# hellovuong/ORB_SLAM3_FAST

Hardware: AMD Instinct MI355X
Metric: ORB extract+match frames/sec @1280×720 stereo (both-eye ORBextractor + ComputeStereoMatches) (higher is better)
Workload: dtype u8; 1 GPU; C3: synthetic 1280x720 rectified stereo pairs, 1500 features, 8 levels, scale 1.2, FAST 20/7, ComputeStereoMatches (bf=0.12*532.03, b=0.12); handles=4, distinct_streams_per_gpu=32, frames_in_ring=3, stereo_matches_pair0=987, parallelism=independent stereo pairs sharded across GPUs, no data-path collective

## Files before the change

### include/orbx.h

```cpp
#ifndef ORBX_H_
#define ORBX_H_

#include <stddef.h>
#include <stdint.h>

#ifdef __cplusplus
extern "C" {
#endif

#define ORBX_MAX_LEVELS 12

#define ORBX_OK 0
#define ORBX_E_EMPTY (-1)
#define ORBX_E_BADARG (-2)
#define ORBX_E_CAPACITY (-3)
#define ORBX_E_HIP (-4)
#define ORBX_E_NODEVICE (-5)
#define ORBX_E_UNSUPPORTED (-6)
#define ORBX_E_TIMEOUT (-7)

typedef struct orbx_keypoint {
  float x, y, size, angle, response;
  int32_t octave, class_id;
} orbx_keypoint;
// ... 576 lines not shown
int orbx_copy_probe(int device, size_t bytes, int iters, double* gbps);

void orbx_debug_introsort(uint64_t* v, int n);
int orbx_debug_introsort_device(int device, uint64_t* v, int n);

void orbx_debug_set_detect_list_cap(int cap);
void orbx_debug_set_octree_global(int on);
void orbx_debug_set_stereo_direct(int max_pairs);
int orbx_debug_upload_results(orbx_extractor* ex, int image, const orbx_keypoint* kps, const uint8_t* desc, int n, int mono_index);
void orbx_debug_set_clahe_cell_kernel(int on);
void orbx_debug_set_remap_lds(int on);
int orbx_debug_remap_footprints(const float* map_x, const float* map_y, ptrdiff_t map_stride, int out_w, int out_h, int src_w,
                                int src_h, int n_maps, int32_t* table, int cap, int32_t* tiles_x, int32_t* tiles_y);
int orbx_debug_front_tables(const orbx_params* p, int width, int height, uint32_t* cells, int cells_cap, uint32_t* tiles,
                            int tiles_cap, int32_t info[4]);
int orbx_debug_preproc_plan(const orbx_preproc* pp, int32_t info[8]);
void orbx_debug_set_resize_tail(int first_level, int max_levels, int band_rows);
int orbx_debug_resize_plan(const orbx_extractor* ex, int32_t* first_level, int32_t* n_levels, int32_t* n_bands, int cap);
int orbx_debug_score_map(orbx_extractor* ex, int enable);
int orbx_debug_score_level(orbx_extractor* ex, int image, int level, uint8_t* dst, ptrdiff_t dst_stride);
int orbx_debug_sincos(int device, const float* angles, int n, int fused, float* sin_out, float* cos_out);

#ifdef __cplusplus
}
#endif
#endif
```

### orb_slam3_fast_amd/__init__.py

```python
import ctypes as C
import os

import numpy as np

_HERE = os.path.dirname(os.path.abspath(__file__))
LIB_PATH = os.path.join(_HERE, os.environ.get("ORBX_LIB_NAME", "liborbx.so"))

KP_DTYPE = np.dtype([("x", "<f4"), ("y", "<f4"), ("size", "<f4"), ("angle", "<f4"), ("response", "<f4"),
                     ("octave", "<i4"), ("class_id", "<i4")])
assert KP_DTYPE.itemsize == 28

OK, E_EMPTY, E_BADARG, E_CAPACITY, E_HIP, E_NODEVICE, E_UNSUPPORTED, E_TIMEOUT = 0, -1, -2, -3, -4, -5, -6, -7
TH_HIGH, TH_LOW, HISTO_LENGTH = 100, 50, 30
NUM_STAGES = 8
MP_DTYPE = np.dtype([("proj_x", "<f4"), ("proj_y", "<f4"), ("proj_xr", "<f4"), ("view_cos", "<f4"), ("track_depth", "<f4"),
                     ("predicted_level", "<i4"), ("in_view", "u1"), ("bad", "u1"), ("has_observations", "u1"),
                     ("pad_", "u1"), ("desc", "u1", (32,))])
assert MP_DTYPE.itemsize == 60
PP_DTYPE = np.dtype([("u", "<f4"), ("v", "<f4"), ("ur", "<f4"), ("radius", "<f4"), ("angle", "<f4"), ("min_level", "<i4"),
                     ("max_level", "<i4"), ("valid", "u1"), ("has_observations", "u1"), ("pad_", "u1", (2,)),
                     ("desc", "u1", (32,))])
assert PP_DTYPE.itemsize == 64
FP_DTYPE = np.dtype([("u", "<f4"), ("v", "<f4"), ("ur", "<f4"), ("radius", "<f4"), ("predicted_level", "<i4"), ("valid", "u1"),
                     ("pad_", "u1", (3,)), ("desc", "u1", (32,))])
# ... 170 lines not shown
        L.orbx_debug_set_detect_list_cap.argtypes = [i]
        L.orbx_debug_set_detect_list_cap.restype = None
        L.orbx_debug_set_octree_global.argtypes = [i]
        L.orbx_debug_set_octree_global.restype = None
        L.orbx_debug_set_stereo_direct.argtypes = [i]
        L.orbx_debug_set_stereo_direct.restype = None
        L.orbx_debug_set_clahe_cell_kernel.argtypes = [i]
        L.orbx_debug_set_clahe_cell_kernel.restype = None
        L.orbx_debug_upload_results.argtypes = [vp, i, vp, vp, i, i]
        L.orbx_debug_set_remap_lds.argtypes = [i]
        L.orbx_debug_set_remap_lds.restype = None
        L.orbx_debug_remap_footprints.argtypes = [vp, vp, C.c_ssize_t, i, i, i, i, i, vp, i, C.POINTER(i), C.POINTER(i)]
        L.orbx_debug_preproc_plan.argtypes = [vp, vp]
        if hasattr(L, "orbx_debug_front_tables"):
            L.orbx_debug_front_tables.argtypes = [vp, i, i, vp, i, vp, i, vp]
        L.orbx_debug_set_resize_tail.argtypes = [i, i, i]
        L.orbx_debug_set_resize_tail.restype = None
        L.orbx_debug_resize_plan.argtypes = [vp, vp, vp, vp, i]
        L.orbx_debug_sincos.argtypes = [i, vp, i, i, vp, vp]
        L.orbx_debug_score_map.argtypes = [vp, i]
        L.orbx_set_opencv_compat.argtypes = [vp, i]
        L.orbx_debug_score_level.argtypes = [vp, i, i, vp, C.c_ssize_t]
        _lib = L
    return _lib


def _check(rc):
    if rc < 0:
        raise OrbxError(rc, lib().orbx_last_error().decode())
    return rc
# ... 1090 lines not shown
        raise OrbxError("unexpected tile grid %d x %d" % (gx.value, gy.value))
    return tab if rc == 1 else None


def front_tables(nfeatures, scaleFactor, nlevels, iniThFAST, minThFAST, width, height):
    prm = _Params(int(nfeatures), float(scaleFactor), int(nlevels), int(iniThFAST), int(minThFAST))
    info = np.zeros(4, np.int32)
    _check(lib().orbx_debug_front_tables(C.byref(prm), width, height, None, 0, None, 0, _p(info)))
    cells = np.zeros((int(info[0]), 16), np.uint32)
    tiles = np.zeros(int(info[1]), np.uint32)
    _check(lib().orbx_debug_front_tables(C.byref(prm), width, height, _p(cells), cells.size, _p(tiles) if tiles.size else None,
                                         tiles.size, _p(info)))
    return cells, tiles, int(info[2]), int(info[3])


class ORBVocabulary:

    def __init__(self, k=None, L=None, parent=None, is_leaf=None, desc=None, weight=None, scoring=0, weighting=0, path=None,
                 device=0):
        h = C.c_void_p()
        if path is not None:
            _check(lib().orbx_vocabulary_load_text(device, path.encode(), C.byref(h)))
        else:
            parent = np.ascontiguousarray(parent, np.int32)
            leaf = np.ascontiguousarray(is_leaf, np.uint8)
            d = np.ascontiguousarray(desc, np.uint8)
            w = np.ascontiguousarray(weight, np.float64)
            _check(lib().orbx_vocabulary_create(device, k, L, scoring, weighting, len(parent), _p(parent), _p(leaf), _p(d), _p(w),
                                                C.byref(h)))
        self._h = h
# ... 491 lines not shown
```

### orb_slam3_fast_amd/csrc/orbx_api.hip

```cpp
#include "orbx_host.h"
#include "orbx_rgbd.h"

namespace orbx_host {
thread_local std::string g_err;
}

namespace {
struct StageTimer {
  orbx_extractor* ex;
  hipStream_t s;
  int stage;
  size_t i0 = 0;
  bool on;
  StageTimer(orbx_extractor* ex_, hipStream_t s_, int stage_)
      : ex(ex_), s(s_), stage(stage_), on(ex_->profiling && (ex_->profStage < 0 || ex_->profStage == stage_)) {
    if (!on) {
      if (s == ex->stream) ex->lastEvValid = false;
      return;
    }
    if (s == ex->stream && ex->lastEvValid) {
      i0 = ex->lastEv;
    } else {
      hipEvent_t e = ex->next_event();
      i0 = ex->evCursor - 1;
// ... 175 lines not shown
        t[3] = (uint32_t)cb | ((uint32_t)ndw << 16);
        t[4] = (fast ? kTileFast : 0u) | (whole ? kTileWhole : 0u);
        t[5] = (uint32_t)((long long)y0 * D.pitch);
        t[6] = (uint32_t)tby;
      }
      for (int w = 0; w < 4; w++)
        for (int k = 0; k < 4; k++) {
          const int dy = std::min(y0 + w + 4 * k, D.h - 1);
          const uint32_t sy = yrow[D.ycoef + dy];
          uint32_t* r = &tab[(size_t)rowOff + 16 * (size_t)(4 * tby + w) + 4 * k];
          r[0] = (uint32_t)(uint16_t)yab[2 * (D.ycoef + dy)] | ((uint32_t)(uint16_t)yab[2 * (D.ycoef + dy) + 1] << 16);
          r[1] = (uint32_t)(((int)(sy & 0xFFFFu) - rb) * 512);
          r[2] = (uint32_t)(((int)(sy >> 16) - rb) * 512);
        }
    }
  }
}

void build_cell_records(const Geom& g, std::vector<CellRec>& recs) {
  recs.assign((size_t)g.totalCells, CellRec{});
  const int TPd = g.tileP >> 2;
  for (int l = 0; l < g.nlevels; l++) {
    const LevelDev& L = g.lv[l];
    const int maxBX = L.w - kBorder, maxBY = L.h - kBorder;
    for (int ci = 0; ci < L.nRows; ci++)
      for (int cj = 0; cj < L.nCols; cj++) {
        const int cell = ci * L.nCols + cj;
        CellRec& r = recs[(size_t)L.cellStart + cell];
        const int iniY = kBorder + ci * L.hCell, iniX = kBorder + cj * L.wCell;
        const int maxY = std::min(iniY + L.hCell + 6, maxBY), maxX = std::min(iniX + L.wCell + 6, maxBX);
// ... 225 lines not shown
  g.cellImg = m.cellImg;
  std::vector<uint4> xtab;
  std::vector<int> yofs;
  std::vector<short> yab;
  build_coefs(g, xtab, yofs, yab);
  HIPC(hipStreamSynchronize(ex->stream));
  HIPC(hipMemcpy(ex->d_xtab.p, xtab.data(), xtab.size() * sizeof(uint4), hipMemcpyHostToDevice));
  HIPC(hipMemcpy(ex->d_yofs.p, yofs.data(), yofs.size() * sizeof(int), hipMemcpyHostToDevice));
  {
    std::vector<uint32_t> yrow, rec;
    build_yrow(g, yofs, yrow);
    HIPC(hipMemcpy(ex->d_yrow.p, yrow.data(), yrow.size() * sizeof(uint32_t), hipMemcpyHostToDevice));
    build_resize_records(g, xtab, yrow, yab, rec);
    if (ex->d_rsRec.n < rec.size()) HIPC(ex->d_rsRec.alloc(rec.size()));
    if (!rec.empty()) HIPC(hipMemcpy(ex->d_rsRec.p, rec.data(), rec.size() * sizeof(uint32_t), hipMemcpyHostToDevice));
  }
  HIPC(hipMemcpy(ex->d_yab.p, yab.data(), yab.size() * sizeof(short), hipMemcpyHostToDevice));
  {
    std::vector<CellRec> recs;
    build_cell_records(g, recs);
    HIPC(hipMemcpy(ex->d_cellRec.p, recs.data(), recs.size() * sizeof(CellRec), hipMemcpyHostToDevice));
  }
  HIPC(prepare_kernels(g));
  std::vector<TailPlan> plans;
  std::vector<TailBand> bands;
  build_tail_plans(g, yofs, plans, bands);
  if (!plans.empty()) {
    if (ex->d_tailBands.n < bands.size()) HIPC(ex->d_tailBands.alloc(bands.size()));
    HIPC(hipMemcpy(ex->d_tailBands.p, bands.data(), bands.size() * sizeof(TailBand), hipMemcpyHostToDevice));
    unsigned lds = 0;
// ... 92 lines not shown
  if (ex->useLat) {
    for (const TailPlan& tp : ex->latTails) {
      StageTimer t(ex, s, ORBX_STAGE_RESIZE);
      HIPC(launch_resize_tail(g, ex->pyr, tp, ex->d_latBands.p + tp.bandOff, img0, n, ex->d_xtab.p, ex->d_yofs.p, ex->d_yab.p, s));
    }
    return ORBX_OK;
  }
  size_t seg = 0;
  for (int l = 1; l < g.nlevels;) {
    StageTimer t(ex, s, ORBX_STAGE_RESIZE);
    if (seg < ex->tails.size() && ex->tails[seg].lA == l) {
      const TailPlan& tp = ex->tails[seg++];
      HIPC(launch_resize_tail(g, ex->pyr, tp, ex->d_tailBands.p + tp.bandOff, 0, n, ex->d_xtab.p, ex->d_yofs.p, ex->d_yab.p, s));
      l += tp.nT;
    } else {
      HIPC(launch_resize(g, ex->pyr, n, l, ex->d_xtab.p, ex->d_yrow.p, ex->d_yab.p, ex->d_rsRec.p, s));
      l++;
    }
  }
  return ORBX_OK;
}

int enqueue_extract(orbx_extractor* ex, const uint8_t* d_images, int n, int w, int h, ptrdiff_t row_pitch,
                    ptrdiff_t image_pitch, const int32_t* lap) {
  bool lapTrivial = true;
  int rc = prepare_extract(ex, d_images, n, w, h, row_pitch, image_pitch, lap, lapTrivial);
  if (rc != ORBX_OK) return rc;
  hipStream_t s = ex->stream;
  static const bool useGraph = getenv("ORBX_GRAPH") && atoi(getenv("ORBX_GRAPH")) != 0;
  if (useGraph && n == 1 && d_images == ex->d_stage.p && !ex->profiling && !ex->graphOff) {
    if (ex->graphW != w || ex->graphH != h) {
// ... 822 lines not shown
  build_yrow(g, yofs, yrow);
  build_resize_records(g, xtab, yrow, yab, rec);
  build_cell_records(g, cr);
  info[0] = (int32_t)cr.size(); info[1] = (int32_t)rec.size(); info[2] = g.tileP; info[3] = g.tileH;
  if (cells) {
    if (cr.size() * 16 > (size_t)cells_cap) return fail(ORBX_E_CAPACITY, "cell records larger than cells_cap");
    std::memcpy(cells, cr.data(), cr.size() * sizeof(CellRec));
  }
  if (tiles) {
    if (rec.size() > (size_t)tiles_cap) return fail(ORBX_E_CAPACITY, "tile records larger than tiles_cap");
    std::memcpy(tiles, rec.data(), rec.size() * sizeof(uint32_t));
  }
  return ORBX_OK;
}

int orbx_hamming256(const void* a, const void* b) {
  const uint32_t* x = (const uint32_t*)a;
  const uint32_t* y = (const uint32_t*)b;
  int d = 0;
  for (int i = 0; i < 8; i++) d += __builtin_popcount(x[i] ^ y[i]);
  return d;
}

static int enqueue_stereo_match(orbx_extractor* left, int first_left, orbx_extractor* right, int first_right,
                                int n_pairs, float bf, float b, bool withFilter, StereoArgs* argsOut,
                                const ResultPack* packWithBand, bool* packedOut) {
  if (packedOut) *packedOut = false;
  if (!left || !right) return fail(ORBX_E_BADARG, "null handle");
  if (n_pairs <= 0 || first_left < 0 || first_right < 0 || first_left + n_pairs > left->lastN ||
      first_right + n_pairs > right->lastN)
// ... 355 lines not shown
```

### orb_slam3_fast_amd/csrc/orbx_host.h

```cpp
#ifndef ORBX_HOST_H
#define ORBX_HOST_H
#if defined(__x86_64__) || defined(__i386__)
#include <immintrin.h>
static inline void cpu_pause() { _mm_pause(); }
#else
static inline void cpu_pause() {}
#endif
#include <memory>
#include <new>
#include <chrono>
#include <cmath>
#include <cstdio>
#include <cstdlib>
#include <cstring>
#include <string>
#include <mutex>
#include <vector>

#include "orbx_internal.h"

using namespace orbx;

namespace orbx_host {


extern thread_local std::string g_err;
void build_coefs(const Geom& g, std::vector<uint4>& xtab, std::vector<int>& yofs, std::vector<short>& yab);
void build_cell_records(const Geom& g, std::vector<CellRec>& recs);
void build_yrow(const Geom& g, const std::vector<int>& yofs, std::vector<uint32_t>& yrow);
void build_resize_records(const Geom& g, const std::vector<uint4>& xtab, const std::vector<uint32_t>& yrow, const std::vector<short>& yab,
                          std::vector<uint32_t>& tab);
inline int fail(int code, const std::string& msg) {
  g_err = msg;
  return code;
}
inline double trace_slow_ms() {
  static const double v = getenv("ORBX_TRACE_SLOW") ? atof(getenv("ORBX_TRACE_SLOW")) : 0.0;
  return v;
}
#define HIPC(expr)                                                                                     \
  do {                                                                                                 \
    const double lim_ = trace_slow_ms();                                                               \
    const auto t0_ = lim_ > 0 ? std::chrono::steady_clock::now() : std::chrono::steady_clock::time_point(); \
    hipError_t e_ = (expr);                                                                            \
    if (lim_ > 0) {                                                                                    \
      const double ms_ = std::chrono::duration<double, std::milli>(std::chrono::steady_clock::now() - t0_).count(); \
// ... 236 lines not shown
  std::vector<int> nfeat;
  int umax[16];
  Geom g{};
  Geom gmax{};
  int curW = 0, curH = 0;
  Pyr pyr{};
  int lastN = 0;
  DevBuf<uint8_t> d_pyr, d_blur, d_stage, d_desc;
  DevBuf<uint8_t> d_dbgScore;
  DevBuf<uint32_t> d_cand, d_cellCand, d_sel;
  DevBuf<uint16_t> d_knode;
  DevBuf<int> d_rowStart, d_cellCount, d_cellPrefix, d_candCount, d_selCount, d_slot, d_nOut, d_mono, d_lap, d_yofs, d_sad;
  DevBuf<short> d_yab;
  DevBuf<uint4> d_xtab;
  DevBuf<uint32_t> d_rsRec;
  DevBuf<orbx::CellRec> d_cellRec;
  DevBuf<int> d_packCtr;
  uint32_t packSeq = 0;
  bool packCtrDirty = false;
  DevBuf<uint32_t> d_yrow;
  DevBuf<uint4> d_srec, d_sdesc;
  std::vector<orbx::TailPlan> tails;
  DevBuf<orbx::TailBand> d_tailBands;
  std::vector<orbx::TailPlan> latTails;
  DevBuf<orbx::TailBand> d_latBands;
  DevBuf<orbx_keypoint> d_kps;
  DevBuf<float> d_uR, d_depth;
  int stagePitch = 0;
  int stereoPairs = 0;
  int lastStereoPairs = 0;
// ... 94 lines not shown
```

### orb_slam3_fast_amd/csrc/orbx_internal.h

```cpp
#pragma once
#include <hip/hip_runtime.h>
#include <stdint.h>
#include <vector>

#include "../../include/orbx.h"

namespace orbx {

constexpr int kEdge = 19;
constexpr int kHalfPatch = 15;
constexpr int kBorder = 16;
constexpr int kMaxIni = 8;

struct LevelDev {
  int w, h, pitch;
  int nCols, nRows, wCell, hCell;
  int cellStart;
  int quota;
  int candCap;
  int cellCap;
  int selOff, selCap;
  int xcoef, ycoef;
  long long off;
  long long candOff;
// ... 76 lines not shown
  int pitch[ORBX_MAX_LEVELS + 1];
  int rtOff[ORBX_MAX_LEVELS];
  int rtTotal;
  unsigned ldsBytes;
};
hipError_t launch_resize_tail(const Geom& g, const Pyr& p, const TailPlan& tp, const TailBand* bands, int img0, int nimg,
                              const uint4* xtab, const int* yofs, const short* yab, hipStream_t s);
hipError_t prepare_resize_tail(unsigned ldsBytes);
hipError_t raise_dynamic_lds(const void* fn, size_t bytes);

size_t resize_plain_lds(int sw, int sh, int dw, int dh);
hipError_t prepare_resize_plain(int sw, int sh, int dw, int dh);
hipError_t launch_resize_plain(const uint8_t* src, int sw, int sh, long long sp, long long sip, uint8_t* dst, int dw, int dh,
                               long long dp, long long dip, const uint4* xtab, const uint32_t* yrow, const short* yab, int nimg,
                               hipStream_t s);
hipError_t launch_resize(const Geom& g, const Pyr& p, int nimg, int level, const uint4* xtab, const uint32_t* yofs ,
                         const short* yab, const uint32_t* records, hipStream_t s);
int resize_records_layout(const Geom& g, int level, int& tileOff, int& rowOff);
constexpr uint32_t kTileFast = 1u, kTileWhole = 2u;
hipError_t launch_detect(const Geom& g, const Pyr& p, const CellRec* cellRec, int nimg, uint32_t* cellCand, int* cellCount,
                         int level0, int level1, uint8_t* dbgScore, hipStream_t s);
hipError_t launch_octree(const Geom& g, int nimg, const uint32_t* cellCand, const int* cellCount, int* cellPrefix,
                         uint32_t* cand, int* candCount, uint16_t* knode, uint32_t* sel, int* selCount, int level0,
                         int level1, hipStream_t s);
hipError_t launch_blur(const Geom& g, const Pyr& p, int nimg, int level0, int level1, hipStream_t s);
hipError_t launch_slots(const Geom& g, int nimg, const uint32_t* sel, const int* selCount, const int* lap,
                        int* slot, int* nOut, int* mono, hipStream_t s);
hipError_t launch_describe(const Geom& g, const Pyr& p, int nimg, const uint32_t* sel, const int* selCount,
                           const int* slot, orbx_keypoint* kps, uint8_t* desc, int* nOut, int* mono, hipStream_t s);
size_t octree_lds_bytes(const Geom& g);
size_t resize_lds_bytes(const Geom& g);

struct StereoArgs {
// ... 381 lines not shown
```

### orb_slam3_fast_amd/csrc/orbx_kernels.hip

```cpp
#include <type_traits>
#include <map>
#include <mutex>

#include "orbx_device.h"
#include "orbx_introsort.h"
#include "orbx_sincos.h"
#include "orbx_blur_mfma.h"

namespace orbx {

__constant__ int c_umax[16] = {15, 15, 15, 15, 14, 14, 14, 13, 13, 12, 11, 10, 9, 8, 6, 3};

#define RS_DW 256
#define RS_DR 16
#define RS_HROWS 6
struct ResizeLv {
  struct { int w, h, pitch, xcoef, ycoef; } D;
  struct { int w, h; } S;
  int sp, l;
  int nbx;
  const uint8_t* src; long long srcImg;
  uint8_t* dst; long long dstImg;
  const uint32_t* tiles;
  const uint32_t* rows;
};
constexpr int kResizeXcdRun = 8;
__device__ __forceinline__ uint32_t vblend4(uint2 t0, uint2 t1, uint32_t bb, uint32_t kRound) {
  uint32_t p0, p1, p2, p3, q0, q1, q2, q3, w01, w23;
  asm("v_mad_u32_u16 %0, %1, %2, %3" : "=v"(p0) : "v"(t0.x), "s"(bb), "v"(kRound));
  asm("v_mad_u32_u16 %0, %1, %2, %3 op_sel:[1,0,0,0]" : "=v"(p1) : "v"(t0.x), "s"(bb), "v"(kRound));
  asm("v_mad_u32_u16 %0, %1, %2, %3" : "=v"(p2) : "v"(t0.y), "s"(bb), "v"(kRound));
  asm("v_mad_u32_u16 %0, %1, %2, %3 op_sel:[1,0,0,0]" : "=v"(p3) : "v"(t0.y), "s"(bb), "v"(kRound));
  asm("v_mad_u32_u16 %0, %1, %2, 0 op_sel:[0,1,0,0]" : "=v"(q0) : "v"(t1.x), "s"(bb));
  asm("v_mad_u32_u16 %0, %1, %2, 0 op_sel:[1,1,0,0]" : "=v"(q1) : "v"(t1.x), "s"(bb));
  asm("v_mad_u32_u16 %0, %1, %2, 0 op_sel:[0,1,0,0]" : "=v"(q2) : "v"(t1.y), "s"(bb));
  asm("v_mad_u32_u16 %0, %1, %2, 0 op_sel:[1,1,0,0]" : "=v"(q3) : "v"(t1.y), "s"(bb));
  asm("v_add_u32_sdwa %0, %1, %2 dst_sel:WORD_0 dst_unused:UNUSED_PAD src0_sel:WORD_1 src1_sel:WORD_1" : "=v"(w01) : "v"(p0), "v"(q0));
  asm("v_add_u32_sdwa %0, %1, %2 dst_sel:WORD_1 dst_unused:UNUSED_PRESERVE src0_sel:WORD_1 src1_sel:WORD_1" : "+v"(w01) : "v"(p1), "v"(q1));
  asm("v_add_u32_sdwa %0, %1, %2 dst_sel:WORD_0 dst_unused:UNUSED_PAD src0_sel:WORD_1 src1_sel:WORD_1" : "=v"(w23) : "v"(p2), "v"(q2));
  asm("v_add_u32_sdwa %0, %1, %2 dst_sel:WORD_1 dst_unused:UNUSED_PRESERVE src0_sel:WORD_1 src1_sel:WORD_1" : "+v"(w23) : "v"(p3), "v"(q3));
  asm("v_pk_lshrrev_b16 %0, 2, %1 op_sel_hi:[0,1]" : "=v"(w01) : "v"(w01));
  asm("v_pk_lshrrev_b16 %0, 2, %1 op_sel_hi:[0,1]" : "=v"(w23) : "v"(w23));
  return __builtin_amdgcn_perm(w23, w01, 0x06040200u);
}
template <int NDW, bool TAB>
__global__ __launch_bounds__(256) void k_resize(ResizeLv rl, const uint4* __restrict__ xtab,
                                                const uint32_t* __restrict__ yrow, const short* __restrict__ yab,
                                                int srcRowsMax, int srcDwMaxRt) {
  extern __shared__ __attribute__((aligned(16))) uint8_t smem[];
  const int SDW = NDW ? NDW : srcDwMaxRt;
  const auto D = rl.D;
  const auto S = rl.S;
  const int l = rl.l;
  const int tid = threadIdx.x;
  const int img = blockIdx.z;
  const int tIdx = xcd_run_remap<kResizeXcdRun>((int)blockIdx.x, (int)gridDim.x, (int)blockIdx.z);
  const int sp = rl.sp;
  const uint8_t* src = rl.src + (long long)img * rl.srcImg;
  uint32_t* st = reinterpret_cast<uint32_t*>(smem);
  uint8_t* ht8 = smem + (size_t)srcRowsMax * SDW * 4;
#ifdef RS_PROF
  long long tq0 = wall_clock64();
#endif
  const int qc = tid & 63, w = __builtin_amdgcn_readfirstlane(tid >> 6);
  int x0, rowsHere;
  int rb, nrows, cb, ndw;
  bool whole, fastGeom;
  const uint4* xt;
  uint8_t* dstTile;
  uint32_t vbb[RS_DR / 4];
  int vr0[RS_DR / 4], vr1[RS_DR / 4];
  constexpr int kFastTrips = 8;
  if (TAB) {
    const uint32_t* tr = rl.tiles + 8 * tIdx;
    xt = xtab + tr[0];
    x0 = (int)(tr[1] & 0xFFFFu), rowsHere = (int)(tr[1] >> 16);
    rb = (int)(tr[2] & 0xFFFFu), nrows = (int)(tr[2] >> 16);
    cb = (int)(tr[3] & 0xFFFFu), ndw = (int)(tr[3] >> 16);
    whole = (tr[4] & kTileWhole) != 0, fastGeom = (tr[4] & kTileFast) != 0;
    dstTile = rl.dst + (long long)img * rl.dstImg + tr[5];
    const uint4* rw4 = reinterpret_cast<const uint4*>(rl.rows) + (4 * (int)tr[6] + w) * (RS_DR / 4);
#pragma unroll
    for (int k = 0; k < RS_DR / 4; k++) {
      const uint4 e = rw4[k];
      vbb[k] = e.x, vr0[k] = (int)e.y, vr1[k] = (int)e.z;
    }
  } else {
    const int tby = __builtin_amdgcn_readfirstlane((int)(((float)tIdx + 0.5f) * __builtin_amdgcn_rcpf((float)rl.nbx)));
    const int tbx = tIdx - tby * rl.nbx;
    const int y0 = tby * RS_DR;
    x0 = tbx * RS_DW;
    const int x1 = min(x0 + RS_DW, D.w) - 1, y1 = min(y0 + RS_DR, D.h) - 1;
    rowsHere = y1 - y0 + 1;
    rb = (int)(yrow[D.ycoef + y0] & 0xFFFFu);
    nrows = (int)(yrow[D.ycoef + y1] >> 16) - rb + 1;
    cb = (int)xtab[D.xcoef + x0].y;
    const int ce = min((int)xtab[D.xcoef + x1].x + 1, S.w - 1);
    ndw = ((ce - cb) >> 2) + 1;
    whole = l > 1 || cb + 4 * ndw <= S.w;
// ... 16 lines not shown
    ba[j] = (int)e.y - cb;
    sel[j] = e.z;
    coef[j] = e.w;
  }
  {
    if (NDW != 0 && fastGeom) {
      const float inv_nd = __builtin_amdgcn_rcpf((float)ndw);
      const int r0 = (int)(((float)tid + 0.5f) * inv_nd);
      const int c = tid - __mul24(r0, ndw);
      const uint8_t* fb = src + (long long)rb * sp + cb;
      const uint32_t off0 = (uint32_t)(__mul24(r0, sp) + 4 * c);
      uint8_t* sdst = smem + 4 * (__mul24(r0, NDW) + c);
      uint32_t v[kFastTrips];
      const uint8_t* fbk[kFastTrips];
#pragma unroll
      for (int k = 0; k < kFastTrips; k++) fbk[k] = fb + (size_t)(3 * k) * (size_t)sp;
      static_assert(kFastTrips == 8, "the asm below issues eight loads");
      asm volatile(
          "global_load_dword %0, %8, %9\n\t"
          "global_load_dword %1, %8, %10\n\t"
          "global_load_dword %2, %8, %11\n\t"
          "global_load_dword %3, %8, %12\n\t"
          "global_load_dword %4, %8, %13\n\t"
          "global_load_dword %5, %8, %14\n\t"
          "global_load_dword %6, %8, %15\n\t"
          "global_load_dword %7, %8, %16\n\t"
          "s_waitcnt vmcnt(0)"
          : "=&v"(v[0]), "=&v"(v[1]), "=&v"(v[2]), "=&v"(v[3]), "=&v"(v[4]), "=&v"(v[5]), "=&v"(v[6]), "=&v"(v[7])
          : "v"(off0), "s"(fbk[0]), "s"(fbk[1]), "s"(fbk[2]), "s"(fbk[3]), "s"(fbk[4]), "s"(fbk[5]), "s"(fbk[6]), "s"(fbk[7])
          : "memory");
#pragma unroll
// ... 119 lines not shown
  srcRowsMax = (int)((double)RS_DR * S.h / D.h) + 4;
  srcDwMax = ((int)((double)RS_DW * S.w / D.w) + 12) / 4 + 1;
  lds = (size_t)srcRowsMax * srcDwMax * 4 + (size_t)srcRowsMax * RS_DW * 2;
}
size_t resize_lds_bytes(const Geom& g) {
  size_t m = 0;
  for (int l = 1; l < g.nlevels; l++) {
    int a, b;
    size_t n;
    resize_footprint(g, l, a, b, n);
    m = n > m ? n : m;
  }
  return m;
}

constexpr int kResizeNdw = 80;
int resize_records_layout(const Geom& g, int level, int& tileOff, int& rowOff) {
  int n = 0;
  tileOff = rowOff = 0;
  for (int l = 1; l < g.nlevels && l <= level; l++) {
    const int nbx = (g.lv[l].w + RS_DW - 1) / RS_DW, nby = (g.lv[l].h + RS_DR - 1) / RS_DR;
    tileOff = n;
    rowOff = n + 8 * nbx * nby;
    n = rowOff + 4 * RS_DR * nby;
  }
  return n;
}

hipError_t launch_resize(const Geom& g, const Pyr& p, int nimg, int level, const uint4* xtab, const uint32_t* yofs,
                         const short* yab, const uint32_t* records, hipStream_t s) {
  const LevelDev& D = g.lv[level];
  int srcRowsMax, srcDwMax;
  size_t lds;
  resize_footprint(g, level, srcRowsMax, srcDwMax, lds);
  const int nbx = (D.w + RS_DW - 1) / RS_DW, nby = (D.h + RS_DR - 1) / RS_DR;
  dim3 grid(nbx * nby, 1, nimg);
  const LevelDev& S = g.lv[level - 1];
  ResizeLv rl;
  rl.nbx = nbx;
  rl.tiles = rl.rows = nullptr;
  if (records) {
    int tileOff, rowOff;
    resize_records_layout(g, level, tileOff, rowOff);
    rl.tiles = records + tileOff;
    rl.rows = records + rowOff;
  }
  rl.D.w = D.w; rl.D.h = D.h; rl.D.pitch = D.pitch; rl.D.xcoef = D.xcoef; rl.D.ycoef = D.ycoef;
  rl.S.w = S.w; rl.S.h = S.h;
  rl.l = level;
  if (level == 1) {
    rl.sp = (int)p.l0Row; rl.src = p.l0; rl.srcImg = p.l0Img;
  } else {
    rl.sp = S.pitch; rl.src = p.pyr + S.off; rl.srcImg = g.pyrImg;
  }
  rl.dst = p.pyr + D.off; rl.dstImg = g.pyrImg;
  auto go = [&](auto kern) { hipLaunchKernelGGL(kern, grid, dim3(256), lds, s, rl, xtab, yofs, yab, srcRowsMax, srcDwMax); };
  if (srcDwMax == kResizeNdw) {
    if (records) go(k_resize<kResizeNdw, true>); else go(k_resize<kResizeNdw, false>);
  } else {
    if (records) go(k_resize<0, true>); else go(k_resize<0, false>);
// ... 12 lines not shown
  return g;
}
size_t resize_plain_lds(int sw, int sh, int dw, int dh) { return resize_lds_bytes(resize_plain_geom(sw, sh, dw, dh, 0, 0)); }
hipError_t prepare_resize_plain(int sw, int sh, int dw, int dh) {
  const size_t lds = std::max<size_t>(resize_plain_lds(sw, sh, dw, dh), 1024);
  hipError_t e = raise_dynamic_lds(reinterpret_cast<const void*>(k_resize<0, false>), lds);
  if (e == hipSuccess) e = raise_dynamic_lds(reinterpret_cast<const void*>(k_resize<kResizeNdw, false>), lds);
  return e;
}
hipError_t launch_resize_plain(const uint8_t* src, int sw, int sh, long long sp, long long sip, uint8_t* dst, int dw, int dh,
                               long long dp, long long dip, const uint4* xtab, const uint32_t* yrow, const short* yab, int nimg,
                               hipStream_t s) {
  const Geom g = resize_plain_geom(sw, sh, dw, dh, dp, dip);
  Pyr p{};
  p.l0 = src; p.l0Row = sp; p.l0Img = sip; p.pyr = dst;
  return launch_resize(g, p, nimg, 1, xtab, yrow, yab, nullptr, s);
}


__device__ __forceinline__ void wsync() {
  __builtin_amdgcn_fence(__ATOMIC_SEQ_CST, "wavefront");
  __builtin_amdgcn_wave_barrier();
}

__device__ int partition_wave(uint64_t* a, int first, int last, uint16_t* Li, uint16_t* Ri, int lane) {
  const KeyLess less;
  const int mid = first + (last - first) / 2;
  {
    const uint64_t va = a[first + 1], vb = a[mid], vc = a[last - 1];
    int sel;
    if (less(va, vb)) sel = less(vb, vc) ? mid : (less(va, vc) ? last - 1 : first + 1);
// ... 2105 lines not shown
```

Before: 83930 stereo frames/s.

## Pack ragged right-edge resize tiles into multi-row-band strip blocks

Adds a per-level strip table so the narrow last column of 256-wide resize tiles is handled by blocks that pack several 16-row bands across the wavefront, with lanes split into (subrow, quad) groups. Full tiles are remapped with a magic-multiply that skips the last column, and the grid shrinks to full tiles plus strips. This aims to cut the mostly idle lanes and extra block launches spent on thin edge tiles, at the cost of a more complex kernel path. Table reads also move to the constant address space for scalar loads.

```diff
diff --git a/include/orbx.h b/include/orbx.h
--- a/include/orbx.h
+++ b/include/orbx.h
@@ -614,6 +614,7 @@
                                 int src_h, int n_maps, int32_t* table, int cap, int32_t* tiles_x, int32_t* tiles_y);
 int orbx_debug_front_tables(const orbx_params* p, int width, int height, uint32_t* cells, int cells_cap, uint32_t* tiles,
                             int tiles_cap, int32_t info[4]);
+int orbx_debug_resize_strips(const orbx_params* p, int width, int height, uint32_t* strips, int strips_cap, int32_t info[2]);
 int orbx_debug_preproc_plan(const orbx_preproc* pp, int32_t info[8]);
 void orbx_debug_set_resize_tail(int first_level, int max_levels, int band_rows);
 int orbx_debug_resize_plan(const orbx_extractor* ex, int32_t* first_level, int32_t* n_levels, int32_t* n_bands, int cap);
diff --git a/orb_slam3_fast_amd/__init__.py b/orb_slam3_fast_amd/__init__.py
--- a/orb_slam3_fast_amd/__init__.py
+++ b/orb_slam3_fast_amd/__init__.py
@@ -208,6 +208,8 @@
         L.orbx_debug_preproc_plan.argtypes = [vp, vp]
         if hasattr(L, "orbx_debug_front_tables"):
             L.orbx_debug_front_tables.argtypes = [vp, i, i, vp, i, vp, i, vp]
+        if hasattr(L, "orbx_debug_resize_strips"):
+            L.orbx_debug_resize_strips.argtypes = [vp, i, i, vp, i, vp]
         L.orbx_debug_set_resize_tail.argtypes = [i, i, i]
         L.orbx_debug_set_resize_tail.restype = None
         L.orbx_debug_resize_plan.argtypes = [vp, vp, vp, vp, i]
@@ -1328,6 +1330,15 @@
     return cells, tiles, int(info[2]), int(info[3])
 
 
+def resize_strips(nfeatures, scaleFactor, nlevels, iniThFAST, minThFAST, width, height):
+    prm = _Params(int(nfeatures), float(scaleFactor), int(nlevels), int(iniThFAST), int(minThFAST))
+    info = np.zeros(2, np.int32)
+    _check(lib().orbx_debug_resize_strips(C.byref(prm), width, height, None, 0, _p(info)))
+    tab = np.zeros(int(info[0]), np.uint32)
+    _check(lib().orbx_debug_resize_strips(C.byref(prm), width, height, _p(tab) if tab.size else None, tab.size, _p(info)))
+    return tab
+
+
 class ORBVocabulary:
 
     def __init__(self, k=None, L=None, parent=None, is_leaf=None, desc=None, weight=None, scoring=0, weighting=0, path=None,
diff --git a/orb_slam3_fast_amd/csrc/orbx_api.hip b/orb_slam3_fast_amd/csrc/orbx_api.hip
--- a/orb_slam3_fast_amd/csrc/orbx_api.hip
+++ b/orb_slam3_fast_amd/csrc/orbx_api.hip
@@ -213,6 +213,84 @@
           r[2] = (uint32_t)(((int)(sy >> 16) - rb) * 512);
         }
     }
+  }
+}
+
+void build_resize_strips(const Geom& g, const std::vector<uint4>& xtab, const std::vector<uint32_t>& yrow, const std::vector<short>& yab,
+                         std::vector<uint32_t>& tab, ResizeStrips* lv) {
+  const int nl = g.nlevels;
+  tab.assign((size_t)8 * std::max(nl - 1, 0), 0u);
+  for (int l = 1; l < nl; l++) {
+    const LevelDev &D = g.lv[l], &S = g.lv[l - 1];
+    ResizeStrips& R = lv[l];
+    R = ResizeStrips{};
+    const int nbx = (D.w + 255) / 256, nby = (D.h + 15) / 16;
+    const int x0 = (nbx - 1) * 256, x1 = D.w - 1;
+    const int q = (x1 - x0) / 4 + 1;
+    R.q = q;
+    R.nFull = nbx * nby;
+    const int cb = (int)xtab[D.xcoef + x0].y;
+    const int ce = std::min((int)xtab[D.xcoef + x1].x + 1, S.w - 1);
+    const int ndw = ((ce - cb) >> 2) + 1;
+    const bool whole = l > 1 || cb + 4 * ndw <= S.w;
+    const size_t ldsMax = resize_level_lds(g, l);
+    const int m = nbx - 1;
+    const uint32_t mul = m > 0 ? (uint32_t)((65536 + m - 1) / m) : 0u;
+    bool mulOk = (long long)m * nby < 65536;
+    for (int t = 0; mulOk && t < m * nby; t++) mulOk = (int)(((uint32_t)t * mul) >> 16) == t / m;
+    auto need = [&](int r, int y0) {
+      const int y1 = std::min(y0 + 16 * r, D.h) - 1;
+      const int nrows = (int)(yrow[D.ycoef + y1] >> 16) - (int)(yrow[D.ycoef + y0] & 0xFFFFu) + 1;
+      return (((size_t)nrows * ndw * 4 + 7) & ~(size_t)7) + (size_t)nrows * q * 8;
+    };
+    int r = 0;
+    if (q <= 32 && mulOk) {
+      for (r = 64 / q; r >= 1; r--) {
+        size_t worst = 0;
+        for (int y0 = 0; y0 < D.h; y0 += 16 * r) worst = std::max(worst, need(r, y0));
+        if (worst <= ldsMax) {
+          R.ldsBytes = (int)worst;
+          break;
+        }
+      }
+    }
+    if (r >= 1) {
+      R.r = r;
+      R.n = (D.h + 16 * r - 1) / (16 * r);
+      R.nFull = m * nby;
+      R.tbyMul = mul;
+      R.recOff = (int)tab.size();
+      R.rowOff = R.recOff + 8 * R.n;
+      tab.resize((size_t)R.rowOff + (size_t)R.n * 16 * r * 4, 0u);
+      for (int i = 0; i < R.n; i++) {
+        const int y0 = i * 16 * r, y1 = std::min(y0 + 16 * r, D.h) - 1;
+        const int rb = (int)(yrow[D.ycoef + y0] & 0xFFFFu), nrows = (int)(yrow[D.ycoef + y1] >> 16) - rb + 1;
+        uint32_t* t = &tab[(size_t)R.recOff + 8 * (size_t)i];
+        t[0] = (uint32_t)(D.xcoef + x0);
+        t[1] = (uint32_t)x0 | ((uint32_t)(y1 - y0 + 1) << 16);
+        t[2] = (uint32_t)rb | ((uint32_t)nrows << 16);
+        t[3] = (uint32_t)cb | ((uint32_t)ndw << 16);
+        t[4] = (whole ? kTileWhole : 0u) | ((uint32_t)q << 8) | ((uint32_t)r << 16);
+        t[5] = (uint32_t)((long long)y0 * D.pitch);
+        t[6] = (uint32_t)(i * 16 * r);
+        t[7] = (uint32_t)y0;
+        for (int w = 0; w < 4; w++)
+          for (int k = 0; k < 4; k++)
+            for (int sr = 0; sr < r; sr++) {
+              const int row = (4 * k + w) * r + sr;
+              const int dy = std::min(y0 + row, y1);
+              const uint32_t sy = yrow[D.ycoef + dy];
+              uint32_t* e = &tab[(size_t)R.rowOff + 4 * ((size_t)i * 16 * r + (size_t)(4 * w + k) * r + sr)];
+              e[0] = (uint32_t)(uint16_t)yab[2 * (D.ycoef + dy)] | ((uint32_t)(uint16_t)yab[2 * (D.ycoef + dy) + 1] << 16);
+              e[1] = (uint32_t)(((int)(sy & 0xFFFFu) - rb) * 8 * q);
+              e[2] = (uint32_t)(((int)(sy >> 16) - rb) * 8 * q);
+              e[3] = y0 + row <= y1 ? (uint32_t)((long long)dy * D.pitch) : 0xFFFFFFFFu;
+            }
+      }
+    }
+    uint32_t* h = &tab[(size_t)8 * (l - 1)];
+    h[0] = (uint32_t)R.q; h[1] = (uint32_t)R.r; h[2] = (uint32_t)R.n; h[3] = (uint32_t)R.nFull;
+    h[4] = R.tbyMul; h[5] = (uint32_t)R.recOff; h[6] = (uint32_t)R.rowOff; h[7] = (uint32_t)R.ldsBytes;
   }
 }
 
@@ -468,6 +546,9 @@
     build_resize_records(g, xtab, yrow, yab, rec);
     if (ex->d_rsRec.n < rec.size()) HIPC(ex->d_rsRec.alloc(rec.size()));
     if (!rec.empty()) HIPC(hipMemcpy(ex->d_rsRec.p, rec.data(), rec.size() * sizeof(uint32_t), hipMemcpyHostToDevice));
+    build_resize_strips(g, xtab, yrow, yab, rec, ex->rsStrips);
+    if (ex->d_rsStrip.n < rec.size()) HIPC(ex->d_rsStrip.alloc(rec.size()));
+    if (!rec.empty()) HIPC(hipMemcpy(ex->d_rsStrip.p, rec.data(), rec.size() * sizeof(uint32_t), hipMemcpyHostToDevice));
   }
   HIPC(hipMemcpy(ex->d_yab.p, yab.data(), yab.size() * sizeof(short), hipMemcpyHostToDevice));
   {
@@ -590,7 +671,7 @@
       HIPC(launch_resize_tail(g, ex->pyr, tp, ex->d_tailBands.p + tp.bandOff, 0, n, ex->d_xtab.p, ex->d_yofs.p, ex->d_yab.p, s));
       l += tp.nT;
     } else {
-      HIPC(launch_resize(g, ex->pyr, n, l, ex->d_xtab.p, ex->d_yrow.p, ex->d_yab.p, ex->d_rsRec.p, s));
+      HIPC(launch_resize(g, ex->pyr, n, l, ex->d_xtab.p, ex->d_yrow.p, ex->d_yab.p, ex->d_rsRec.p, ex->d_rsStrip.p, &ex->rsStrips[l], s));
       l++;
     }
   }
@@ -1443,6 +1524,32 @@
   return ORBX_OK;
 }
 
+int orbx_debug_resize_strips(const orbx_params* p, int width, int height, uint32_t* strips, int strips_cap, int32_t info[2]) {
+  if (!p || !info || width < 1 || height < 1 || strips_cap < 0 || (strips_cap && !strips) || p->nlevels < 1 ||
+      p->nlevels > ORBX_MAX_LEVELS || p->nfeatures < 1 || !(p->scale_factor > 1.0f))
+    return fail(ORBX_E_BADARG, "bad argument");
+  std::unique_ptr<orbx_extractor> ex(new orbx_extractor());
+  ex->prm = *p;
+  build_tables(ex.get());
+  Geom g;
+  std::string why;
+  const int rc = build_geom(ex.get(), width, height, g, why);
+  if (rc != ORBX_OK) return fail(rc, why);
+  std::vector<uint4> xtab;
+  std::vector<int> yofs;
+  std::vector<short> yab;
+  std::vector<uint32_t> yrow, tab;
+  build_coefs(g, xtab, yofs, yab);
+  build_yrow(g, yofs, yrow);
+  build_resize_strips(g, xtab, yrow, yab, tab, ex->rsStrips);
+  info[0] = (int32_t)tab.size(); info[1] = g.nlevels - 1;
+  if (strips) {
+    if (tab.size() > (size_t)strips_cap) return fail(ORBX_E_CAPACITY, "strip table larger than strips_cap");
+    std::memcpy(strips, tab.data(), tab.size() * sizeof(uint32_t));
+  }
+  return ORBX_OK;
+}
+
 int orbx_hamming256(const void* a, const void* b) {
   const uint32_t* x = (const uint32_t*)a;
   const uint32_t* y = (const uint32_t*)b;
diff --git a/orb_slam3_fast_amd/csrc/orbx_host.h b/orb_slam3_fast_amd/csrc/orbx_host.h
--- a/orb_slam3_fast_amd/csrc/orbx_host.h
+++ b/orb_slam3_fast_amd/csrc/orbx_host.h
@@ -30,6 +30,8 @@
 void build_yrow(const Geom& g, const std::vector<int>& yofs, std::vector<uint32_t>& yrow);
 void build_resize_records(const Geom& g, const std::vector<uint4>& xtab, const std::vector<uint32_t>& yrow, const std::vector<short>& yab,
                           std::vector<uint32_t>& tab);
+void build_resize_strips(const Geom& g, const std::vector<uint4>& xtab, const std::vector<uint32_t>& yrow, const std::vector<short>& yab,
+                         std::vector<uint32_t>& tab, ResizeStrips* lv);
 inline int fail(int code, const std::string& msg) {
   g_err = msg;
   return code;
@@ -296,6 +298,8 @@
   DevBuf<short> d_yab;
   DevBuf<uint4> d_xtab;
   DevBuf<uint32_t> d_rsRec;
+  DevBuf<uint32_t> d_rsStrip;
+  ResizeStrips rsStrips[ORBX_MAX_LEVELS] = {};
   DevBuf<orbx::CellRec> d_cellRec;
   DevBuf<int> d_packCtr;
   uint32_t packSeq = 0;
diff --git a/orb_slam3_fast_amd/csrc/orbx_internal.h b/orb_slam3_fast_amd/csrc/orbx_internal.h
--- a/orb_slam3_fast_amd/csrc/orbx_internal.h
+++ b/orb_slam3_fast_amd/csrc/orbx_internal.h
@@ -114,9 +114,17 @@
 hipError_t launch_resize_plain(const uint8_t* src, int sw, int sh, long long sp, long long sip, uint8_t* dst, int dw, int dh,
                                long long dp, long long dip, const uint4* xtab, const uint32_t* yrow, const short* yab, int nimg,
                                hipStream_t s);
+struct ResizeStrips {
+  int q, r;
+  int n, nFull;
+  uint32_t tbyMul;
+  int recOff, rowOff;
+  int ldsBytes;
+};
 hipError_t launch_resize(const Geom& g, const Pyr& p, int nimg, int level, const uint4* xtab, const uint32_t* yofs ,
-                         const short* yab, const uint32_t* records, hipStream_t s);
+                         const short* yab, const uint32_t* records, const uint32_t* strips, const ResizeStrips* sl, hipStream_t s);
 int resize_records_layout(const Geom& g, int level, int& tileOff, int& rowOff);
+size_t resize_level_lds(const Geom& g, int level);
 constexpr uint32_t kTileFast = 1u, kTileWhole = 2u;
 hipError_t launch_detect(const Geom& g, const Pyr& p, const CellRec* cellRec, int nimg, uint32_t* cellCand, int* cellCount,
                          int level0, int level1, uint8_t* dbgScore, hipStream_t s);
diff --git a/orb_slam3_fast_amd/csrc/orbx_kernels.hip b/orb_slam3_fast_amd/csrc/orbx_kernels.hip
--- a/orb_slam3_fast_amd/csrc/orbx_kernels.hip
+++ b/orb_slam3_fast_amd/csrc/orbx_kernels.hip
@@ -23,8 +23,17 @@
   uint8_t* dst; long long dstImg;
   const uint32_t* tiles;
   const uint32_t* rows;
+  const uint32_t* strips;
+  const uint4* stripRows;
+  int nFull;
+  uint32_t tbyMul;
 };
 constexpr int kResizeXcdRun = 8;
+typedef uint32_t u32x4 __attribute__((ext_vector_type(4)));
+template <class T>
+__device__ __forceinline__ const __attribute__((address_space(4))) T* const_tab(const T* p) {
+  return (const __attribute__((address_space(4))) T*)p;
+}
 __device__ __forceinline__ uint32_t vblend4(uint2 t0, uint2 t1, uint32_t bb, uint32_t kRound) {
   uint32_t p0, p1, p2, p3, q0, q1, q2, q3, w01, w23;
   asm("v_mad_u32_u16 %0, %1, %2, %3" : "=v"(p0) : "v"(t0.x), "s"(bb), "v"(kRound));
@@ -43,6 +52,139 @@
   asm("v_pk_lshrrev_b16 %0, 2, %1 op_sel_hi:[0,1]" : "=v"(w23) : "v"(w23));
   return __builtin_amdgcn_perm(w23, w01, 0x06040200u);
 }
+__device__ __forceinline__ uint32_t vblend4v(uint2 t0, uint2 t1, uint32_t bb, uint32_t kRound) {
+  uint32_t p0, p1, p2, p3, q0, q1, q2, q3, w01, w23;
+  asm("v_mad_u32_u16 %0, %1, %2, %3" : "=v"(p0) : "v"(t0.x), "v"(bb), "v"(kRound));
+  asm("v_mad_u32_u16 %0, %1, %2, %3 op_sel:[1,0,0,0]" : "=v"(p1) : "v"(t0.x), "v"(bb), "v"(kRound));
+  asm("v_mad_u32_u16 %0, %1, %2, %3" : "=v"(p2) : "v"(t0.y), "v"(bb), "v"(kRound));
+  asm("v_mad_u32_u16 %0, %1, %2, %3 op_sel:[1,0,0,0]" : "=v"(p3) : "v"(t0.y), "v"(bb), "v"(kRound));
+  asm("v_mad_u32_u16 %0, %1, %2, 0 op_sel:[0,1,0,0]" : "=v"(q0) : "v"(t1.x), "v"(bb));
+  asm("v_mad_u32_u16 %0, %1, %2, 0 op_sel:[1,1,0,0]" : "=v"(q1) : "v"(t1.x), "v"(bb));
+  asm("v_mad_u32_u16 %0, %1, %2, 0 op_sel:[0,1,0,0]" : "=v"(q2) : "v"(t1.y), "v"(bb));
+  asm("v_mad_u32_u16 %0, %1, %2, 0 op_sel:[1,1,0,0]" : "=v"(q3) : "v"(t1.y), "v"(bb));
+  asm("v_add_u32_sdwa %0, %1, %2 dst_sel:WORD_0 dst_unused:UNUSED_PAD src0_sel:WORD_1 src1_sel:WORD_1" : "=v"(w01) : "v"(p0), "v"(q0));
+  asm("v_add_u32_sdwa %0, %1, %2 dst_sel:WORD_1 dst_unused:UNUSED_PRESERVE src0_sel:WORD_1 src1_sel:WORD_1" : "+v"(w01) : "v"(p1), "v"(q1));
+  asm("v_add_u32_sdwa %0, %1, %2 dst_sel:WORD_0 dst_unused:UNUSED_PAD src0_sel:WORD_1 src1_sel:WORD_1" : "=v"(w23) : "v"(p2), "v"(q2));
+  asm("v_add_u32_sdwa %0, %1, %2 dst_sel:WORD_1 dst_unused:UNUSED_PRESERVE src0_sel:WORD_1 src1_sel:WORD_1" : "+v"(w23) : "v"(p3), "v"(q3));
+  asm("v_pk_lshrrev_b16 %0, 2, %1 op_sel_hi:[0,1]" : "=v"(w01) : "v"(w01));
+  asm("v_pk_lshrrev_b16 %0, 2, %1 op_sel_hi:[0,1]" : "=v"(w23) : "v"(w23));
+  return __builtin_amdgcn_perm(w23, w01, 0x06040200u);
+}
+__device__ __forceinline__ void resize_strip(const ResizeLv& rl, const uint4* __restrict__ xtab, int sIdx, int img, uint8_t* smem) {
+  const int tid = threadIdx.x;
+  const int lane = tid & 63, w = __builtin_amdgcn_readfirstlane(tid >> 6);
+  const auto* tr = const_tab(rl.strips + 8 * sIdx);
+  const uint4* xt = xtab + tr[0];
+  const int x0 = (int)(tr[1] & 0xFFFFu), rowsHere = (int)(tr[1] >> 16);
+  const int rb = (int)(tr[2] & 0xFFFFu), nrows = (int)(tr[2] >> 16);
+  const int cb = (int)(tr[3] & 0xFFFFu), ndw = (int)(tr[3] >> 16);
+  const bool whole = (tr[4] & kTileWhole) != 0;
+  const int q = (int)((tr[4] >> 8) & 0xFFu), r = (int)(tr[4] >> 16);
+  const int sp = rl.sp;
+  const uint8_t* src = rl.src + (long long)img * rl.srcImg;
+  uint8_t* dstLv = rl.dst + (long long)img * rl.dstImg;
+  const int s = (int)(((float)lane + 0.5f) * __builtin_amdgcn_rcpf((float)q));
+  const int quad = lane - s * q;
+  const bool act = s < r;
+  uint4 ent[RS_DR / 4];
+  {
+    const uint4* re = rl.stripRows + tr[6] + 4 * w * r + min(s, r - 1);
+#pragma unroll
+    for (int k = 0; k < RS_DR / 4; k++) ent[k] = re[k * r];
+  }
+  uint32_t sel[4], coef[4];
+  int ba[4];
+#pragma unroll
+  for (int j = 0; j < 4; j++) {
+    const uint4 e = xt[4 * quad + j];
+    ba[j] = (int)e.y - cb;
+    sel[j] = e.z;
+    coef[j] = e.w;
+  }
+  uint32_t* st = reinterpret_cast<uint32_t*>(smem);
+  {
+    const float inv_nd = __builtin_amdgcn_rcpf((float)ndw);
+    const int rpp = __builtin_amdgcn_readfirstlane((int)(256.5f * inv_nd));
+    const int r0 = (int)(((float)tid + 0.5f) * inv_nd);
+    const int c = tid - r0 * ndw;
+    constexpr int kTrips = 8;
+    if (whole) {
+      const uint8_t* fb = src + (long long)rb * sp + cb;
+      const uint32_t offLast = (uint32_t)(__mul24(nrows - 1, sp) + 4 * c), offStep = (uint32_t)(rpp * sp);
+      const int idxLast = 4 * (__mul24(nrows - 1, ndw) + c), idxStep = 4 * rpp * ndw;
+      for (int rbase = 0; rbase < nrows; rbase += rpp * kTrips) {
+        const uint32_t off0 = (uint32_t)(__mul24(rbase + r0, sp) + 4 * c);
+        const int idx0 = 4 * (__mul24(rbase + r0, ndw) + c);
+        uint32_t v[kTrips];
+#pragma unroll
+        for (int k = 0; k < kTrips; k++) v[k] = *reinterpret_cast<const uint32_t*>(fb + min(off0 + (uint32_t)k * offStep, offLast));
+#pragma unroll
+        for (int k = 0; k < kTrips; k++) *reinterpret_cast<uint32_t*>(smem + min(idx0 + k * idxStep, idxLast)) = v[k];
+      }
+    } else {
+      const bool lanes = r0 < rpp;
+      const int gx = cb + 4 * c;
+      const bool wide = gx + 4 <= rl.S.w;
+      for (int rbase = 0; rbase < nrows; rbase += rpp * kTrips) {
+        uint32_t v[kTrips];
+        const uint8_t* p = src + (long long)(rb + rbase + r0) * sp + gx;
+#pragma unroll
+        for (int k = 0; k < kTrips; k++) {
+          v[k] = 0;
+          if (lanes && rbase + r0 + k * rpp < nrows) {
+            if (wide) {
+              v[k] = *reinterpret_cast<const uint32_t*>(p);
+            } else {
+              for (int bI = 0; bI < 4; bI++)
+                if (gx + bI < rl.S.w) v[k] |= (uint32_t)p[bI] << (8 * bI);
+            }
+          }
+          p += (long long)rpp * sp;
+        }
+#pragma unroll
+        for (int k = 0; k < kTrips; k++)
+          if (lanes && rbase + r0 + k * rpp < nrows) st[(rbase + r0 + k * rpp) * ndw + c] = v[k];
+      }
+    }
+  }
+  __syncthreads();
+  uint8_t* ht8 = smem + ((nrows * ndw * 4 + 7) & ~7);
+  const int hp = 8 * q;
+  for (int g = w; g * r < nrows; g += 4) {
+    const int row = g * r + s;
+    if (act && row < nrows) {
+      const uint8_t* rowp = smem + row * ndw * 4;
+      uint32_t t[4];
+#pragma unroll
+      for (int j = 0; j < 4; j++) {
+        const uint32_t* pr = reinterpret_cast<const uint32_t*>(rowp + ba[j]);
+        t[j] = udot2_u16(__builtin_amdgcn_perm(pr[1], pr[0], sel[j]), coef[j], 0u);
+      }
+      uint2 pk;
+      pk.x = (t[0] >> 4) | ((t[1] >> 4) << 16);
+      pk.y = (t[2] >> 4) | ((t[3] >> 4) << 16);
+      *reinterpret_cast<uint2*>(ht8 + row * hp + 8 * quad) = pk;
+    }
+  }
+  __syncthreads();
+  uint32_t kRound = 0x20000u;
+  asm volatile("" : "+v"(kRound));
+  if (act) {
+    const uint8_t* htq = ht8 + 8 * quad;
+    const uint32_t dx = (uint32_t)(x0 + 4 * quad);
+#pragma unroll
+    for (int k = 0; k < RS_DR / 4; k++) {
+      if ((4 * k + w) * r >= rowsHere) break;
+      const uint4 e = ent[k];
+      if (e.w != 0xFFFFFFFFu) {
+        const uint2 t0 = *reinterpret_cast<const uint2*>(htq + e.y);
+        const uint2 t1 = *reinterpret_cast<const uint2*>(htq + e.z);
+        const uint32_t outw = vblend4v(t0, t1, e.x, kRound);
+        asm volatile("global_store_dword %0, %1, %2" : : "v"(e.w + dx), "v"(outw), "s"(dstLv) : "memory");
+      }
+    }
+  }
+}
 template <int NDW, bool TAB>
 __global__ __launch_bounds__(256) void k_resize(ResizeLv rl, const uint4* __restrict__ xtab,
                                                 const uint32_t* __restrict__ yrow, const short* __restrict__ yab,
@@ -55,6 +197,10 @@
   const int tid = threadIdx.x;
   const int img = blockIdx.z;
   const int tIdx = xcd_run_remap<kResizeXcdRun>((int)blockIdx.x, (int)gridDim.x, (int)blockIdx.z);
+  if (TAB && tIdx >= rl.nFull) {
+    resize_strip(rl, xtab, tIdx - rl.nFull, img, smem);
+    return;
+  }
   const int sp = rl.sp;
   const uint8_t* src = rl.src + (long long)img * rl.srcImg;
   uint32_t* st = reinterpret_cast<uint32_t*>(smem);
@@ -72,17 +218,17 @@
   int vr0[RS_DR / 4], vr1[RS_DR / 4];
   constexpr int kFastTrips = 8;
   if (TAB) {
-    const uint32_t* tr = rl.tiles + 8 * tIdx;
+    const auto* tr = const_tab(rl.tiles + 8 * (tIdx + (int)(((uint32_t)tIdx * rl.tbyMul) >> 16)));
     xt = xtab + tr[0];
     x0 = (int)(tr[1] & 0xFFFFu), rowsHere = (int)(tr[1] >> 16);
     rb = (int)(tr[2] & 0xFFFFu), nrows = (int)(tr[2] >> 16);
     cb = (int)(tr[3] & 0xFFFFu), ndw = (int)(tr[3] >> 16);
     whole = (tr[4] & kTileWhole) != 0, fastGeom = (tr[4] & kTileFast) != 0;
     dstTile = rl.dst + (long long)img * rl.dstImg + tr[5];
-    const uint4* rw4 = reinterpret_cast<const uint4*>(rl.rows) + (4 * (int)tr[6] + w) * (RS_DR / 4);
+    const auto* rw4 = const_tab(reinterpret_cast<const u32x4*>(rl.rows) + (4 * (int)tr[6] + w) * (RS_DR / 4));
 #pragma unroll
     for (int k = 0; k < RS_DR / 4; k++) {
-      const uint4 e = rw4[k];
+      const u32x4 e = rw4[k];
       vbb[k] = e.x, vr0[k] = (int)e.y, vr1[k] = (int)e.z;
     }
   } else {
@@ -129,7 +275,7 @@
       uint32_t v[kFastTrips];
       const uint8_t* fbk[kFastTrips];
 #pragma unroll
-      for (int k = 0; k < kFastTrips; k++) fbk[k] = fb + (size_t)(3 * k) * (size_t)sp;
+      for (int k = 0; k < kFastTrips; k++) fbk[k] = k ? fbk[k - 1] + (size_t)3 * (size_t)sp : fb;
       static_assert(kFastTrips == 8, "the asm below issues eight loads");
       asm volatile(
           "global_load_dword %0, %8, %9\n\t"
@@ -279,6 +425,13 @@
   return m;
 }
 
+size_t resize_level_lds(const Geom& g, int level) {
+  int a, b;
+  size_t n;
+  resize_footprint(g, level, a, b, n);
+  return n;
+}
+
 constexpr int kResizeNdw = 80;
 int resize_records_layout(const Geom& g, int level, int& tileOff, int& rowOff) {
   int n = 0;
@@ -293,7 +446,7 @@
 }
 
 hipError_t launch_resize(const Geom& g, const Pyr& p, int nimg, int level, const uint4* xtab, const uint32_t* yofs,
-                         const short* yab, const uint32_t* records, hipStream_t s) {
+                         const short* yab, const uint32_t* records, const uint32_t* strips, const ResizeStrips* sl, hipStream_t s) {
   const LevelDev& D = g.lv[level];
   int srcRowsMax, srcDwMax;
   size_t lds;
@@ -303,12 +456,23 @@
   const LevelDev& S = g.lv[level - 1];
   ResizeLv rl;
   rl.nbx = nbx;
-  rl.tiles = rl.rows = nullptr;
+  rl.tiles = rl.rows = rl.strips = nullptr;
+  rl.stripRows = nullptr;
+  rl.nFull = nbx * nby;
+  rl.tbyMul = 0;
   if (records) {
     int tileOff, rowOff;
     resize_records_layout(g, level, tileOff, rowOff);
     rl.tiles = records + tileOff;
     rl.rows = records + rowOff;
+    if (strips && sl && sl->n > 0) {
+      if ((size_t)sl->ldsBytes > lds) return hipErrorInvalidValue;
+      rl.strips = strips + sl->recOff;
+      rl.stripRows = reinterpret_cast<const uint4*>(strips + sl->rowOff);
+      rl.nFull = sl->nFull;
+      rl.tbyMul = sl->tbyMul;
+      grid.x = (unsigned)(sl->nFull + sl->n);
+    }
   }
   rl.D.w = D.w; rl.D.h = D.h; rl.D.pitch = D.pitch; rl.D.xcoef = D.xcoef; rl.D.ycoef = D.ycoef;
   rl.S.w = S.w; rl.S.h = S.h;
@@ -351,7 +515,7 @@
   const Geom g = resize_plain_geom(sw, sh, dw, dh, dp, dip);
   Pyr p{};
   p.l0 = src; p.l0Row = sp; p.l0Img = sip; p.pyr = dst;
-  return launch_resize(g, p, nimg, 1, xtab, yrow, yab, nullptr, s);
+  return launch_resize(g, p, nimg, 1, xtab, yrow, yab, nullptr, nullptr, nullptr, s);
 }
 
 
```

Result: faster. 84940 stereo frames/s, median of 6 (+1.2%).
